# JaehaKim97/EDTR

Measured on AMD Instinct MI355X. Metric: restored 512x512 images/sec @ 4 denoise steps, higher is better.
Workload: dtype bf16; 1 GPU; EDTR-det s4 (sd21): vae_encode + q_sample(t=200) + 4 x (ControlNet+UNet) + vae_decode, batch 8/GPU of 512x512; global_batch=8, image_size=512, denoise_steps=4, parallelism=batch-sharded x1, graphs=True, batches_in_flight=2, precision=fast

## Files before the change

edtr_amd/csrc/igemm.hip:

```cpp
#include <stdlib.h>
#include <type_traits>
#include "common.h"

#ifdef EDTR_STAMPS
#define STAMP_VALUE 0
#define EDTR_STAMP(i)                                                                                                  \
    do {                                                                                                               \
        if (threadIdx.x == 0 && p.workspace && p.splitk <= 1) {                                                        \
            uint64_t* sb__ = static_cast<uint64_t*>(p.workspace) +                                                     \
                             (size_t)(blockIdx.x + gridDim.x * (blockIdx.y + gridDim.y * blockIdx.z)) * 16;             \
            if ((i) == 5) sb__[5] = (uint64_t)__builtin_amdgcn_s_getreg(63492) | ((uint64_t)__builtin_amdgcn_s_getreg(63508) << 32); \
            else if ((i) == 6 || (i) == 7) sb__[i] = __builtin_amdgcn_s_memrealtime();                             \
            else if ((i) >= 8) sb__[i] = (uint64_t)(STAMP_VALUE);                                             \
            else sb__[i] = __builtin_amdgcn_s_memtime();                                                               \
        }                                                                                                              \
    } while (0)
#define EDTR_STAMP_T(i)                                                                                                \
    do {                                                                                                               \
        if (threadIdx.x == 0 && p.workspace && p.splitk <= 1) {                                                        \
            uint64_t* sb__ = static_cast<uint64_t*>(p.workspace) +                                                     \
                             (size_t)(blockIdx.x + gridDim.x * (blockIdx.y + gridDim.y * blockIdx.z)) * 16;             \
            sb__[i] = __builtin_amdgcn_s_memtime();                                                                    \
        }                                                                                                              \
    } while (0)
// ... 1148 lines not shown
#pragma unroll
            for (int ni = 0; ni < NI; ++ni)
                bf[ni] = *reinterpret_cast<const U4*>(sw + tile_off(wn * 64 + ni * 32 + l31, c));
#pragma unroll
            for (int mi = 0; mi < MI; ++mi)
#pragma unroll
                for (int ni = 0; ni < NI; ++ni) acc[mi][ni] = T::mfma(af[mi], bf[ni], acc[mi][ni]);
        }
        asm volatile("s_waitcnt lgkmcnt(0)" ::: "memory");
#ifdef EDTR_STAMPS
        stamp_acc[3] += __builtin_amdgcn_s_memtime() - ts2;
#endif
        __builtin_amdgcn_s_barrier();
        asm volatile("" ::: "memory");
    }
    if (nkt == 0) __syncthreads();
    EDTR_STAMP(3);
#ifdef EDTR_STAMPS
#undef STAMP_VALUE
#define STAMP_VALUE stamp_acc[0]
    EDTR_STAMP(8);
#undef STAMP_VALUE
#define STAMP_VALUE stamp_acc[1]
    EDTR_STAMP(9);
#undef STAMP_VALUE
#define STAMP_VALUE stamp_acc[2]
    EDTR_STAMP(10);
#undef STAMP_VALUE
#define STAMP_VALUE stamp_acc[3]
    EDTR_STAMP(11);
#undef STAMP_VALUE
#define STAMP_VALUE 0
#endif
    tile_epilogue<T, MI, NI>(p, acc, smem, m0, n0, o_zoff);
    EDTR_STAMP(4); EDTR_STAMP(7);
}

template <typename T, bool SPATIAL, bool FAST>
int launch_dma(const edtr_igemm_params& p, hipStream_t stream) {
    constexpr int lds = 2 * (128 + 128) * BK * 2;
    static EdtrLdsOnce attr_set;
    if (int rc_ = edtr_lds_attr(reinterpret_cast<const void*>(&igemm_dma_kernel<T, SPATIAL, FAST>), lds, attr_set)) return rc_;
    const int nbm = (p.M + 127) / 128, nbn = (p.N + 127) / 128;
    dim3 grid(nbm * nbn, p.splitk > 1 ? p.splitk : 1, p.Z);
    hipLaunchKernelGGL((igemm_dma_kernel<T, SPATIAL, FAST>), grid, dim3(kThreads), lds, stream, p);
    EDTR_LAUNCH_CHECK();
    if (p.splitk > 1) return launch_splitk_reducer<T>(p, stream);
    return EDTR_OK;
}


struct KState { int t, tap, c0; };

template <typename T, bool SPATIAL>
__global__ void __launch_bounds__(512, 1) igemm_256_kernel(const edtr_igemm_params p) {
    constexpr int HALF = 128 * BK * 2;
    constexpr int BUF = 4 * HALF;
    extern __shared__ __attribute__((aligned(16))) char smem[];

    const int tid = threadIdx.x, lane = tid & 63, wave = __builtin_amdgcn_readfirstlane(tid >> 6);
    const int wr = wave >> 2, wc = wave & 3;
    const int l15 = lane & 15, lq = lane >> 4;

    const int nbm = (p.M + 255) / 256, nbn = (p.N + 255) / 256;
    int bid = blockIdx.x;
    {
        const int nblk = nbm * nbn, q = nblk >> 3, r = nblk & 7, x = bid & 7, j = bid >> 3;
        bid = (x < r ? x * (q + 1) : r * (q + 1) + (x - r) * q) + j;
    }
    int tm, tn;
    tile_coords(p, bid, nbm, nbn, tm, tn);
    const int m0 = tm * 256, n0 = tn * 256;

    const int z = blockIdx.z, zo = z / p.zdiv, zi = z - zo * p.zdiv;
    const int64_t a_zoff = zo * p.a_zs_outer + zi * p.a_zs_inner;
    const int64_t w_zoff = zo * p.w_zs_outer + zi * p.w_zs_inner;
    const int64_t o_zoff = zo * p.o_zs_outer + zi * p.o_zs_inner;
    const uint16_t* a1 = static_cast<const uint16_t*>(p.a1) + a_zoff;
    const uint16_t* wp = static_cast<const uint16_t*>(p.w) + w_zoff;
    const uint32_t smem_base = __builtin_amdgcn_readfirstlane(lds_addr_of(smem));

    const int rsub = lane >> 3, slot = lane & 7;
    const int Cin = p.C1;
    const int LH = p.upsample2x ? p.IH * 2 : p.IH, LW = p.upsample2x ? p.IW * 2 : p.IW;
    const int nvalid = p.n_valid > 0 ? p.n_valid : p.N;
    uint32_t voff_a[4], voff_w[4], a_mask[4], a_par[4];
    int b0 = 0, oy0 = 0, ox0 = 0;
    float rcp_ow = 0.0f, rcp_oh = 0.0f;
    if (SPATIAL) {
        const int hw = p.OH * p.OW;
        b0 = m0 / hw;
        const int rem0 = m0 - b0 * hw;
        oy0 = rem0 / p.OW;
        ox0 = rem0 - oy0 * p.OW;
        rcp_ow = 1.0f / (float)p.OW;
        rcp_oh = 1.0f / (float)p.OH;
    }
    const int64_t a_bias = SPATIAL ? ((int64_t)p.pad_t * p.IW + p.pad_l) * p.ld1 * 2 : 0;
    const u32x4 srd_a = make_srd(reinterpret_cast<const char*>(a1) - a_bias);
    const u32x4 srd_w = make_srd(wp);
#pragma unroll
    for (int q = 0; q < 4; ++q) {
        const int rih = wave * 16 + 8 * (q & 1) + rsub;
        const int row = (q >> 1) * 128 + rih;
        const int coff = (slot ^ ((rih >> 1) & 7)) * 8;
        const int m = m0 + row;
        const bool ok = m < p.M;
        uint32_t mask = 0;
        a_par[q] = 0;
        if (SPATIAL) {
            const int x = ox0 + row;
            int qx = (int)((float)x * rcp_ow), ox = x - qx * p.OW;
            if (ox >= p.OW) { ++qx; ox -= p.OW; }
            if (ox < 0) { --qx; ox += p.OW; }
            const int y = oy0 + qx;
            int qy = (int)((float)y * rcp_oh), oy = y - qy * p.OH;
            if (oy >= p.OH) { ++qy; oy -= p.OH; }
            if (oy < 0) { --qy; oy += p.OH; }
            const int iy0 = oy * p.stride - p.pad_t, ix0 = ox * p.stride - p.pad_l;
            const int ly = iy0 + p.pad_t, lx = ix0 + p.pad_l;
            const int sy = p.upsample2x ? ly >> 1 : ly, sx = p.upsample2x ? lx >> 1 : lx;
            a_par[q] = p.upsample2x ? (uint32_t)((ly & 1) | ((lx & 1) << 1)) : 0u;
            const int64_t pc = (int64_t)(b0 + qy) * p.IH * p.IW + (int64_t)sy * p.IW + sx;
            voff_a[q] = (uint32_t)((pc * p.ld1 + coff) * 2);
            if (p.taps == 9) {
                uint32_t rb = 0, cbits = 0;
#pragma unroll
                for (int k = 0; k < 3; ++k) {
                    const int iy = iy0 + k, ix = ix0 + k;
                    rb |= (iy >= 0 && iy < LH) ? (1u << (3 * k)) : 0u;
                    cbits |= (ix >= 0 && ix < LW) ? (1u << k) : 0u;
                }
                mask = ok ? rb * cbits : 0u;
            } else {
                mask = (ok && ly >= 0 && ly < LH && lx >= 0 && lx < LW) ? 1u : 0u;
            }
        } else {
            voff_a[q] = ok ? (uint32_t)(((int64_t)m * p.ld1 + coff) * 2) : kOobOffset;
            mask = 1u;
        }
        a_mask[q] = mask;
        const int n = n0 + row;
        voff_w[q] = n < nvalid ? (uint32_t)(((int64_t)n * p.ldw + coff) * 2) : kOobOffset;
    }

    const int nkt = p.K / BK;
    auto advance2 = [&](KState& s) {
        s.t += 2;
        if (SPATIAL) {
            s.tap += 2;
            while (s.tap >= p.taps) { s.tap -= p.taps; s.c0 += BK; }
        }
    };
    auto stage_half = [&](const KState& s, int buf, auto Hc) {
        constexpr int H = decltype(Hc)::value;
        const bool live = s.t < nkt;
        const uint32_t dst = smem_base + buf * BUF + H * HALF + wave * 2048;
        if constexpr (H < 2) {
            uint32_t soff = (uint32_t)s.t * (BK * 2), tapbit = 1u;
            uint32_t dy0 = 0, dy1 = 0, dx0 = 0, dx1 = 0;
            if (SPATIAL) {
                int ky = p.pad_t, kx = p.pad_l;
                if (p.taps == 9) { ky = (s.tap * 11) >> 5; kx = s.tap - 3 * ky; tapbit = 1u << s.tap; }
                if (p.upsample2x) {
                    const int rowb = p.IW * p.ld1 * 2, colb = p.ld1 * 2;
                    dy0 = (uint32_t)((((0 + ky - p.pad_t) >> 1) + p.pad_t) * rowb);
                    dy1 = (uint32_t)((((1 + ky - p.pad_t) >> 1) + p.pad_t) * rowb);
                    dx0 = (uint32_t)((((0 + kx - p.pad_l) >> 1) + p.pad_l) * colb);
                    dx1 = (uint32_t)((((1 + kx - p.pad_l) >> 1) + p.pad_l) * colb);
                    soff = (uint32_t)(s.c0 * 2);
                } else {
                    soff = (uint32_t)(((ky * p.IW + kx) * p.ld1 + s.c0) * 2);
                }
            }
            if (!live) tapbit = 0u;
#pragma unroll
            for (int j = 0; j < 2; ++j) {
                constexpr int q0 = H * 2;
                uint32_t vo = voff_a[q0 + j];
                if (SPATIAL && p.upsample2x) vo += ((a_par[q0 + j] & 1u) ? dy1 : dy0) + ((a_par[q0 + j] & 2u) ? dx1 : dx0);
                vo = (a_mask[q0 + j] & tapbit) ? vo : kOobOffset;
                dma16_buf(vo, srd_a, soff, dst + j * 1024);
            }
        } else {
            const uint32_t soff = SPATIAL ? (uint32_t)((s.tap * Cin + s.c0) * 2) : (uint32_t)s.t * (BK * 2);
#pragma unroll
            for (int j = 0; j < 2; ++j) {
                constexpr int q0 = (H - 2) * 2;
                const uint32_t vo = live ? voff_w[q0 + j] : kOobOffset;
                dma16_buf(vo, srd_w, soff, dst + j * 1024);
            }
        }
    };
    using H0 = std::integral_constant<int, 0>;
    using H1 = std::integral_constant<int, 1>;
    using H2 = std::integral_constant<int, 2>;
    using H3 = std::integral_constant<int, 3>;

    const int a_rd = tile_off(wr * 64 + l15, lq);
    const int b_rd = tile_off(wc * 32 + l15, lq);

    f32x4 acc[2][2][4][2];
#pragma unroll
    for (int i = 0; i < 2; ++i)
#pragma unroll
        for (int j = 0; j < 2; ++j)
#pragma unroll
            for (int a = 0; a < 4; ++a)
#pragma unroll
                for (int b = 0; b < 2; ++b) acc[i][j][a][b] = f32x4{0.0f, 0.0f, 0.0f, 0.0f};
    U4 afr[4][2], bfr[2][2][2];

    auto read_a = [&](int buf, int ah) {
        const char* base = smem + buf * BUF + ah * HALF;
#pragma unroll
        for (int mb = 0; mb < 4; ++mb) {
            afr[mb][0] = *reinterpret_cast<const U4*>(base + a_rd + mb * 2048);
            afr[mb][1] = *reinterpret_cast<const U4*>(base + (a_rd ^ 64) + mb * 2048);
        }
    };
    auto read_b = [&](int buf, auto BHc) {
        constexpr int BH = decltype(BHc)::value;
        const char* base = smem + buf * BUF + (2 + BH) * HALF;
#pragma unroll
        for (int nb = 0; nb < 2; ++nb) {
            bfr[BH][nb][0] = *reinterpret_cast<const U4*>(base + b_rd + nb * 2048);
            bfr[BH][nb][1] = *reinterpret_cast<const U4*>(base + (b_rd ^ 64) + nb * 2048);
        }
    };
    auto mma = [&](auto AHc, auto BHc) {
        constexpr int AH = decltype(AHc)::value, BH = decltype(BHc)::value;
#pragma unroll
        for (int ks = 0; ks < 2; ++ks)
#pragma unroll
            for (int mb = 0; mb < 4; ++mb)
#pragma unroll
                for (int nb = 0; nb < 2; ++nb) acc[AH][BH][mb][nb] = T::mfma16(afr[mb][ks], bfr[BH][nb][ks], acc[AH][BH][mb][nb]);
    };
    auto compute = [&](auto AHc, auto BHc) {
        asm volatile("s_waitcnt vmcnt(6)" ::: "memory");
        __builtin_amdgcn_s_barrier();
        asm volatile("s_waitcnt lgkmcnt(0)" ::: "memory");
        __builtin_amdgcn_sched_barrier(0);
        __builtin_amdgcn_s_setprio(1);
        mma(AHc, BHc);
        __builtin_amdgcn_s_setprio(0);
        __builtin_amdgcn_sched_barrier(0);
        __builtin_amdgcn_s_barrier();
        asm volatile("" ::: "memory");
    };

    KState sE{0, 0, 0}, sO{1, 1, 0};
    if (!SPATIAL || p.taps == 1) { sO.tap = 0; sO.c0 = BK; }
    stage_half(sE, 0, H0{}); stage_half(sE, 0, H1{}); stage_half(sE, 0, H2{}); stage_half(sE, 0, H3{});
    stage_half(sO, 1, H2{}); stage_half(sO, 1, H0{});
    advance2(sE);
    asm volatile("s_waitcnt vmcnt(4)" ::: "memory");
    __builtin_amdgcn_s_barrier();
    if (wr == 1) __builtin_amdgcn_s_barrier();
    asm volatile("" ::: "memory");

    const int niter = (nkt + 1) >> 1;
    for (int it = 0; it < niter; ++it) {
        read_b(0, H0{}); read_a(0, 0); stage_half(sO, 1, H3{}); compute(H0{}, H0{});
        read_b(0, H1{});               stage_half(sO, 1, H1{}); compute(H0{}, H1{}); advance2(sO);
        read_a(0, 1);                  stage_half(sE, 0, H2{}); compute(H1{}, H1{});
                                       stage_half(sE, 0, H0{}); compute(H1{}, H0{});
        read_b(1, H0{}); read_a(1, 0); stage_half(sE, 0, H3{}); compute(H0{}, H0{});
        read_b(1, H1{});               stage_half(sE, 0, H1{}); compute(H0{}, H1{}); advance2(sE);
        read_a(1, 1);                  stage_half(sO, 1, H2{}); compute(H1{}, H1{});
                                       stage_half(sO, 1, H0{}); compute(H1{}, H0{});
    }
    asm volatile("s_waitcnt vmcnt(0)" ::: "memory");
    if (wr == 0) __builtin_amdgcn_s_barrier();
    __syncthreads();

    float* stage = reinterpret_cast<float*>(smem);
    const bool gn_acc = p.gn_partial != nullptr && p.splitk <= 1;
    auto epilogue_pass = [&](auto HPc) {
        constexpr int h = decltype(HPc)::value;
#pragma unroll
        for (int bh = 0; bh < 2; ++bh)
#pragma unroll
            for (int mb = 0; mb < 4; ++mb)
#pragma unroll
                for (int nb = 0; nb < 2; ++nb)
#pragma unroll
                    for (int r = 0; r < 4; ++r)
                        stage[(wr * 64 + mb * 16 + 4 * lq + r) * 256 + bh * 128 + wc * 32 + nb * 16 + l15] = acc[h][bh][mb][nb][r];
        float gs[8], gq[8];
#pragma unroll
        for (int j = 0; j < 8; ++j) { gs[j] = 0.0f; gq[j] = 0.0f; }
        rows_phase<T, 128, 256, false, 512, 0, 256, false>(p, stage, m0 + h * 128, n0, p.N, o_zoff, gn_acc, gs, gq);
        __syncthreads();
        if (gn_acc) {
#pragma unroll
            for (int j = 0; j < 8; ++j) { gs[j] += __shfl_xor(gs[j], 32, 64); gq[j] += __shfl_xor(gq[j], 32, 64); }
            if (lane < 32) {
                float* dst = stage + (wave * 256 + lane * 8) * 2;
#pragma unroll
                for (int j = 0; j < 8; ++j) { dst[2 * j] = gs[j]; dst[2 * j + 1] = gq[j]; }
            }
            __syncthreads();
            if (tid < 256 && n0 + tid < p.N && m0 + h * 128 < p.M) {
                float a = 0.0f, q = 0.0f;
#pragma unroll
                for (int w = 0; w < 8; ++w) { a += stage[(w * 256 + tid) * 2]; q += stage[(w * 256 + tid) * 2 + 1]; }
                float* dst = p.gn_partial + ((int64_t)((m0 >> 7) + h) * gn_ld_of(p) + n0 + tid) * 2;
                dst[0] = a;
                dst[1] = q;
            }
            __syncthreads();
        }
    };
    epilogue_pass(H0{});
    epilogue_pass(H1{});
}

template <typename T, bool SPATIAL>
int launch_256(const edtr_igemm_params& p, hipStream_t stream) {
    constexpr int lds = 2 * 4 * 128 * BK * 2;
    static EdtrLdsOnce attr_set;
    if (int rc_ = edtr_lds_attr(reinterpret_cast<const void*>(&igemm_256_kernel<T, SPATIAL>), lds, attr_set)) return rc_;
    const int nbm = (p.M + 255) / 256, nbn = (p.N + 255) / 256;
    dim3 grid(nbm * nbn, 1, p.Z);
    hipLaunchKernelGGL((igemm_256_kernel<T, SPATIAL>), grid, dim3(512), lds, stream, p);
    EDTR_LAUNCH_CHECK();
    return EDTR_OK;
}

template <typename T, bool SPATIAL, int MB, int NB>
__global__ void __launch_bounds__(kThreads, 2) igemm_n160_kernel(const edtr_igemm_params p) {
    constexpr int BM = 32 * MB, BN = 32 * NB;
    constexpr int A_BYTES = BM * BK * 2, W_BYTES = BN * BK * 2, STAGE = A_BYTES + W_BYTES;
    extern __shared__ __attribute__((aligned(16))) char smem[];
    EDTR_STAMP(0); EDTR_STAMP(6); EDTR_STAMP(5);
    stagger_second_slot(p);

    const int tid = threadIdx.x, lane = tid & 63, wave = __builtin_amdgcn_readfirstlane(tid >> 6);
    const int wm = wave >> 1, wn = wave & 1;
    const int l15 = lane & 15, lq = lane >> 4;

    const int nbm = (p.M + BM - 1) / BM, nbn = (p.N + BN - 1) / BN;
    int bid = blockIdx.x;
    {
        const int nblk = nbm * nbn, q = nblk >> 3, r = nblk & 7, x = bid & 7, j = bid >> 3;
        bid = (x < r ? x * (q + 1) : r * (q + 1) + (x - r) * q) + j;
    }
    int tm, tn;
    tile_coords(p, bid, nbm, nbn, tm, tn);
    const int m0 = tm * BM, n0 = tn * BN;

    const int z = blockIdx.z, zo = z / p.zdiv, zi = z - zo * p.zdiv;
    const int64_t a_zoff = zo * p.a_zs_outer + zi * p.a_zs_inner;
    const int64_t w_zoff = zo * p.w_zs_outer + zi * p.w_zs_inner;
    const int64_t o_zoff = zo * p.o_zs_outer + zi * p.o_zs_inner;
    const uint16_t* a1 = static_cast<const uint16_t*>(p.a1) + a_zoff;
    const uint16_t* wp = static_cast<const uint16_t*>(p.w) + w_zoff;
    const uint32_t smem_base = __builtin_amdgcn_readfirstlane(lds_addr_of(smem));

    const int rsub = lane >> 3, slot = lane & 7;
    const int Cin = p.C1;
    const int LH = p.upsample2x ? p.IH * 2 : p.IH, LW = p.upsample2x ? p.IW * 2 : p.IW;
    const int nvalid = p.n_valid > 0 ? p.n_valid : p.N;
    uint32_t voff_a[MB], voff_w[NB], a_mask[MB], a_par[MB];
    int b0 = 0, oy0 = 0, ox0 = 0;
    float rcp_ow = 0.0f, rcp_oh = 0.0f;
    if (SPATIAL) {
        const int hw = p.OH * p.OW;
        b0 = m0 / hw;
        const int rem0 = m0 - b0 * hw;
        oy0 = rem0 / p.OW;
        ox0 = rem0 - oy0 * p.OW;
        rcp_ow = 1.0f / (float)p.OW;
        rcp_oh = 1.0f / (float)p.OH;
    }
    const int64_t a_bias = SPATIAL ? ((int64_t)p.pad_t * p.IW + p.pad_l) * p.ld1 * 2 : 0;
    const u32x4 srd_a = make_srd(reinterpret_cast<const char*>(a1) - a_bias);
    const u32x4 srd_w = make_srd(wp);
#pragma unroll
    for (int j = 0; j < MB; ++j) {
// ... 515 lines not shown
        __syncthreads();
        if (tid < 128 && n0 + tid < p.N) {
            float a = 0.0f, q = 0.0f;
#pragma unroll
            for (int w = 0; w < 8; ++w) { a += stage[(w * 128 + tid) * 2]; q += stage[(w * 128 + tid) * 2 + 1]; }
            float* dst = p.gn_partial + ((int64_t)(2 * tm) * gn_ld_of(p) + n0 + tid) * 2;
            dst[0] = a;
            dst[1] = q;
            dst[2 * gn_ld_of(p)] = 0.0f;
            dst[2 * gn_ld_of(p) + 1] = 0.0f;
        }
    }
    EDTR_STAMP(4); EDTR_STAMP(7);
}

template <typename T, int GEO>
int launch_halo(const edtr_igemm_params& p, hipStream_t stream) {
    constexpr bool UP2 = GEO == 1;
    constexpr int lds = UP2 ? 256 * 132 * 4 : (GEO == 2 ? 2 * 50 * 1024 + 3 * 128 * BK * 2 + 1024 : 2 * 48 * 1024 + 3 * 128 * BK * 2 + (GEO == 0 ? 2048 : 0));
    static EdtrLdsOnce attr_set;
    if (int rc_ = edtr_lds_attr(reinterpret_cast<const void*>(&igemm_halo_kernel<T, GEO>), lds, attr_set)) return rc_;
    const int nbm = GEO == 2 ? p.M >> 8 : (p.M / (p.OH * p.OW)) * (p.OH >> 4) * (p.OW >> 4), nbn = (p.N + 127) / 128;
    hipLaunchKernelGGL((igemm_halo_kernel<T, GEO>), dim3(nbm * nbn, p.splitk > 1 ? p.splitk : 1, 1), dim3(512), lds, stream, p);
    EDTR_LAUNCH_CHECK();
    if (p.splitk > 1) return launch_splitk_reducer<T>(p, stream);
    return EDTR_OK;
}

static bool igemm_halo_img8(const edtr_igemm_params& p) {
    return !p.upsample2x && p.OH == 8 && p.OW == 8 && p.IH == 8 && p.IW == 8 && (p.M & 255) == 0;
}

static bool igemm_halo_ok(const edtr_igemm_params& p, bool spatial) {
    const int up = p.upsample2x ? 2 : 1;
    if (p.upsample2x == 2 && ((p.IH & 15) || (p.IW & 15) || p.w_phase_stride < (int64_t)p.N * p.ldw || p.ldw < 4 * p.C1)) return false;
    return spatial && p.taps == 9 && p.stride == 1 && p.pad_t == 1 && p.pad_l == 1 && p.C2 == 0 && (p.C1 & 63) == 0 &&
           p.OH == p.IH * up && p.OW == p.IW * up && (((p.OH & 15) == 0 && (p.OW & 15) == 0) || igemm_halo_img8(p)) && p.Z == 1 &&
           p.splitk <= p.C1 / 64 && p.act != EDTR_ACT_GEGLU && p.M == (p.M / (p.OH * p.OW)) * p.OH * p.OW;
}

static bool igemm_fast_addressable(const edtr_igemm_params& p, bool spatial) {
    const int64_t a_rows = spatial ? (int64_t)(p.M / (p.OH * p.OW)) * p.IH * p.IW : p.M;
    const int64_t a_bytes = (a_rows + (spatial ? 3 * (int64_t)p.IW + 3 : 0)) * p.ld1 * 2 + (int64_t)p.K * 2;
    const int64_t w_bytes = (int64_t)p.N * p.ldw * 2 + (int64_t)p.K * 2;
    return a_bytes < 0xF0000000LL && w_bytes < 0xF0000000LL;
}

static int dbg_flags() {
    static int dbg = -1;
    if (dbg < 0) {
        const char* e8 = getenv("EDTR_IGEMM_GENERAL_EPILOGUE");
        const char* e10 = getenv("EDTR_IGEMM_N160_TWO_PASS");
        const char* e12 = getenv("EDTR_IGEMM_GEGLU_SERIAL");
        dbg = ((e8 && e8[0] == '1') ? 1 : 0) | ((e10 && e10[0] == '1') ? 2 : 0) | ((e12 && e12[0] == '1') ? 4 : 0);
    }
    return dbg;
}

template <typename T>
int dispatch(const edtr_igemm_params& p, int tile, bool spatial, hipStream_t s, bool dry) {
    if (tile == 20) {
        if (!spatial || !edtr_halo160_ok(p) || !igemm_fast_addressable(p, spatial)) return EDTR_E_UNSUPPORTED;
        if (dry) return tile;
        return edtr_launch_halo160(p, s);
    }
    if (tile == 21) {
        if (!spatial || !edtr_halo512p_ok(p) || !igemm_fast_addressable(p, spatial)) return EDTR_E_UNSUPPORTED;
        if (dry) return tile;
        return edtr_launch_halo512p(p, s);
    }
    if (tile == 17) {
        if (!spatial || !edtr_halo512_ok(p) || !igemm_fast_addressable(p, spatial)) return EDTR_E_UNSUPPORTED;
        if (dry) return tile;
        return edtr_launch_halo512(p, s);
    }
    if (tile == 16) {
        if (!igemm_halo_ok(p, spatial) || !igemm_fast_addressable(p, spatial)) return EDTR_E_UNSUPPORTED;
        if (dry) return tile;
        if (igemm_halo_img8(p)) return launch_halo<T, 2>(p, s);
        if (p.upsample2x == 2) return launch_halo<T, 3>(p, s);
        return p.upsample2x ? launch_halo<T, 1>(p, s) : launch_halo<T, 0>(p, s);
    }
    if (tile >= 3 && tile <= 14) {
        const bool fast = (!p.upsample2x || (p.stride == 1 && (tile == 3 || tile >= 6))) && igemm_fast_addressable(p, spatial);
        if (tile == 14) {
            if (!fast || p.act == EDTR_ACT_GEGLU || p.gn_partial) return EDTR_E_UNSUPPORTED;
            if (dry) return tile;
            return spatial ? launch_n160<T, true, 8, 1>(p, s) : launch_n160<T, false, 8, 1>(p, s);
        }
        if (tile == 8) {
            if (!fast || p.act == EDTR_ACT_GEGLU) return EDTR_E_UNSUPPORTED;
            if (dry) return tile;
            return spatial ? launch_n160<T, true, 4, 5>(p, s) : launch_n160<T, false, 4, 5>(p, s);
        }
        if (tile == 6) {
            if (!fast || p.splitk > 1 || p.act == EDTR_ACT_GEGLU) return EDTR_E_UNSUPPORTED;
            if (dry) return tile;
            return spatial ? launch_256<T, true>(p, s) : launch_256<T, false>(p, s);
        }
        if (dry) return tile;
        if (!spatial) return fast ? launch_dma<T, false, true>(p, s) : launch_dma<T, false, false>(p, s);
        return fast ? launch_dma<T, true, true>(p, s) : launch_dma<T, true, false>(p, s);
    }
    if (dry) return tile;
    if (tile == 1) return spatial ? launch<T, 2, 2, true>(p, s) : launch<T, 2, 2, false>(p, s);
    return spatial ? launch<T, 1, 1, true>(p, s) : launch<T, 1, 1, false>(p, s);
}

}

namespace {
__global__ void __launch_bounds__(256) gn_finalize_kernel(const float* partial, int tiles_per_image, int C, int groups,
                                                         double* sums) {
    __shared__ double red_s[256], red_q[256];
    const int g = blockIdx.x, b = blockIdx.y, cpg = C / groups;
    const int total = tiles_per_image * cpg;
    double s = 0.0, q = 0.0;
    for (int i = threadIdx.x; i < total; i += 256) {
        const int t = i / cpg, c = g * cpg + (i - t * cpg);
        const float* src = partial + (((int64_t)b * tiles_per_image + t) * C + c) * 2;
        s += (double)src[0];
        q += (double)src[1];
    }
    red_s[threadIdx.x] = s;
    red_q[threadIdx.x] = q;
    __syncthreads();
    for (int o = 128; o > 0; o >>= 1) {
        if (threadIdx.x < o) { red_s[threadIdx.x] += red_s[threadIdx.x + o]; red_q[threadIdx.x] += red_q[threadIdx.x + o]; }
        __syncthreads();
    }
    if (threadIdx.x == 0) {
        sums[((int64_t)b * groups + g) * 2] = red_s[0];
        sums[((int64_t)b * groups + g) * 2 + 1] = red_q[0];
    }
}
}

extern "C" int edtr_gn_finalize(const float* partial, int tiles_per_image, int B, int C, int groups, double* sums,
                                edtr_stream_t stream) {
    if (!partial || !sums) return EDTR_E_NULL;
    if (tiles_per_image <= 0 || B <= 0 || C <= 0 || groups <= 0 || C % groups) return EDTR_E_SHAPE;
    hipLaunchKernelGGL(gn_finalize_kernel, dim3(groups, B), dim3(256), 0, static_cast<hipStream_t>(stream), partial,
                       tiles_per_image, C, groups, sums);
    EDTR_LAUNCH_CHECK();
    return EDTR_OK;
}

namespace {
__global__ void __launch_bounds__(256) gn_table_kernel(const float* partial, int tiles_per_image, const double* sums, int C, int groups,
                                                      int HW, const float* gamma, const float* beta, float eps, float* table) {
    __shared__ double red_s[256], red_q[256];
    const int g = blockIdx.x, b = blockIdx.y, cpg = C / groups;
    double s = 0.0, q = 0.0;
    if (partial) {
        const int total = tiles_per_image * cpg;
// ... 72 lines not shown
        return EDTR_E_ALIGN;
    if ((p.a_zs_outer & 7) || (p.a_zs_inner & 7) || (p.w_zs_outer & 7) || (p.w_zs_inner & 7) ||
        (p.o_zs_outer & 3) || (p.o_zs_inner & 3))
        return EDTR_E_ALIGN;
    if ((p.bias_n && !aligned16(p.bias_n)) || (p.rowvec && (!aligned16(p.rowvec) || (p.rowvec_ld & 3)))) return EDTR_E_ALIGN;
    if (p.n_valid < 0 || p.n_valid > p.N) return EDTR_E_SHAPE;
    if (p.residual && p.Z != 1) return EDTR_E_UNSUPPORTED;
    if (p.rowvec && p.Z != 1) return EDTR_E_UNSUPPORTED;
    if (p.splitk < 0) return EDTR_E_SHAPE;
    if (p.splitk <= 1) p.splitk = 1;
    if (p.splitk > 1) {
        if (p.Z != 1 || p.act == EDTR_ACT_GEGLU) return EDTR_E_UNSUPPORTED;
        if (!p.workspace) return EDTR_E_NULL;
        if (p.workspace_bytes < (int64_t)p.splitk * p.M * p.N * 4 || !aligned16(p.workspace)) return EDTR_E_SHAPE;
        if (p.splitk > (p.K + 63) / 64) return EDTR_E_SHAPE;
    }

    if (p.vt_out) {
        if (p.Z != 1 || p.splitk > 1 || p.act == EDTR_ACT_GEGLU || p.residual || p.rowvec || p.gn_partial || p.out_f32 || spatial)
            return EDTR_E_UNSUPPORTED;
        if (p.rows_per_image <= 0 || (p.rows_per_image & 7) || (p.M & 7) || p.vt_col0 <= 0 || p.vt_col0 >= p.N) return EDTR_E_SHAPE;
        if ((p.vt_ld & 7) || p.vt_ld < p.rows_per_image || !aligned16(p.vt_out)) return EDTR_E_ALIGN;
    }

    if (p.row_stats) {
        if (p.Z != 1 || p.splitk > 1 || p.act == EDTR_ACT_GEGLU || p.vt_out) return EDTR_E_UNSUPPORTED;
        if (p.N & 31) return EDTR_E_SHAPE;
        if (!aligned16(p.row_stats)) return EDTR_E_ALIGN;
    }
    if (p.ln_stats) {
        if (p.Z != 1 || p.splitk > 1 || p.taps != 1 || spatial || p.C2) return EDTR_E_UNSUPPORTED;
        if (!p.ln_c1 || !p.ln_c2) return EDTR_E_NULL;
        if (p.ln_slots <= 0 || p.ln_slots * 32 != p.K || p.ln_C <= 0 || p.ln_C > p.K) return EDTR_E_SHAPE;
        if (!aligned16(p.ln_stats) || !aligned16(p.ln_c1) || !aligned16(p.ln_c2)) return EDTR_E_ALIGN;
    }

    const bool dma_ok = p.C2 == 0 && (p.C1 & 63) == 0;
    int tile = p.tile;
    if (tile == 0) {
        const int64_t big = (int64_t)((p.M + 127) / 128) * ((p.N + 127) / 128) * p.Z;
        tile = dma_ok ? 3 : (big >= 200 ? 1 : 2);
        const int nbn256 = (p.N + 255) / 256;
        const int64_t nb256 = (int64_t)((p.M + 255) / 256) * nbn256 * p.Z;
        static int no_auto = -1;
        if (no_auto < 0) {
            const char* e = getenv("EDTR_IGEMM_NO_AUTO");
            no_auto = e ? atoi(e) : 0;
        }
        const bool pp_ok = dma_ok && p.splitk <= 1 && p.act != EDTR_ACT_GEGLU && (!p.upsample2x || p.stride == 1) &&
                           igemm_fast_addressable(p, spatial);
        const int64_t nb160 = (int64_t)((p.M + 127) / 128) * (p.N / 160) * p.Z;
        if (pp_ok && !(no_auto & (1 << 8)) && p.N % 160 == 0 && nb160 >= 200 && (p.N % 128 != 0 || p.K >= 640))
            tile = 8;
        else if (pp_ok && !(no_auto & (1 << 6)) && p.K >= 1024 && nb256 >= 120 && p.N * 5 >= nbn256 * 256 * 4)
            tile = 6;
        static int halo = -1;
        if (halo < 0) {
            const char* e4 = getenv("EDTR_IGEMM_HALO");
            halo = (e4 && e4[0] == '0') ? 0 : 1;
        }
        if (halo && dma_ok && (p.N & 127) == 0 && igemm_halo_ok(p, spatial) && igemm_fast_addressable(p, spatial) &&
            (int64_t)(p.M >> 8) * (p.N >> 7) * p.splitk >= 48)
            tile = 16;
        static int ragged = -1;
        if (ragged < 0) {
            const char* e6 = getenv("EDTR_IGEMM_HALO_RAGGED");
            ragged = (e6 && e6[0] == '0') ? 0 : 1;
        }
        if (halo && ragged && dma_ok && (p.N & 127) != 0 && p.N > 128 && p.splitk <= 1 && igemm_halo_ok(p, spatial) &&
            igemm_fast_addressable(p, spatial)) {
            const int64_t units = (int64_t)(p.M >> 8) * ((p.N + 127) >> 7);
            if (units >= 48 && units <= 256) tile = 16;
        }
        static int skinny = -1;
        if (skinny < 0) {
            const char* e3 = getenv("EDTR_IGEMM_SKINNY");
            skinny = (e3 && e3[0] == '0') ? 0 : 1;
        }
        if (skinny && tile == 3 && p.N <= 32 && p.M >= 65536 && p.splitk <= 1 && !p.gn_partial && p.act != EDTR_ACT_GEGLU &&
            (!p.upsample2x || p.stride == 1) && igemm_fast_addressable(p, spatial))
            tile = 14;
    }
    static int halo512 = -1;
    if (halo512 < 0) {
        const char* e5 = getenv("EDTR_IGEMM_HALO512");
        halo512 = e5 ? atoi(e5) : 1;
    }
    const bool h512_ok = spatial && (p.C1 & 31) == 0 && edtr_halo512_ok(p) && igemm_fast_addressable(p, spatial);
    const int cus = dry ? 256 : edtr_cu_count();
    if (p.tile == 0 && tile == 16 && halo512 > 0 && h512_ok && (int64_t)(p.M >> 9) * (p.N >> 7) >= (int64_t)cus * halo512) tile = 17;
    static int halo512p = -1;
    if (halo512p < 0) {
        const char* e13 = getenv("EDTR_IGEMM_HALO512P");
        halo512p = e13 ? atoi(e13) : 0;
    }
    if (p.tile == 0 && tile == 17 && halo512p > 0 && edtr_halo512p_ok(p) && (int64_t)(p.M >> 9) * (p.N >> 7) >= (int64_t)cus * halo512p) tile = 21;
    static int halo160 = -1;
    if (halo160 < 0) {
        const char* e10 = getenv("EDTR_IGEMM_HALO160");
        halo160 = (e10 && e10[0] == '0') ? 0 : 1;
    }
    if (p.tile == 0 && tile == 8 && halo160 && spatial && edtr_halo160_ok(p) && igemm_fast_addressable(p, spatial)) {
        const int64_t units = (int64_t)(p.M >> 8) * (p.N / 160), tail = units % cus, most = (int64_t)cus * 3 / 4;
        if (units >= most && (tail == 0 || tail >= most)) tile = 20;
    }
    if (p.a_gn) {
        if (p.tile == 21 || (p.tile == 0 && tile == 21)) {
            if (!h512_ok || !edtr_halo512p_ok(p)) return EDTR_E_UNSUPPORTED;
            tile = 21;
        } else if (p.tile == 17 || (p.tile == 0 && tile == 17)) {
            if (!h512_ok) return EDTR_E_UNSUPPORTED;
            tile = 17;
        } else {
            if ((p.dtype != EDTR_BF16 && p.dtype != EDTR_F16) || !spatial || p.upsample2x || !dma_ok || !igemm_halo_ok(p, spatial) ||
                igemm_halo_img8(p) || !igemm_fast_addressable(p, spatial) || (p.tile != 0 && p.tile != 16))
                return EDTR_E_UNSUPPORTED;
            tile = 16;
        }
        if (!aligned16(p.a_gn)) return EDTR_E_ALIGN;
    }
    if (p.out16) {
        if (!p.out_f32 || p.Z != 1 || p.act == EDTR_ACT_GEGLU || p.vt_out) return EDTR_E_UNSUPPORTED;
        if ((p.ld16 & 7) || !aligned16(p.out16)) return EDTR_E_ALIGN;
    }
    if (p.a_wrap != 0) {
        if (p.a_wrap < 0 || p.K != 2 * p.a_wrap || (p.a_wrap & 63) || spatial || p.taps != 1 || p.C2 || p.Z != 1 || p.ln_stats) return EDTR_E_UNSUPPORTED;
        if (p.tile != 0 && !(p.tile == 1 || p.tile == 2 || p.tile == 3 || p.tile == 8)) return EDTR_E_UNSUPPORTED;
        if (!(tile == 1 || tile == 2 || tile == 3 || tile == 8)) tile = 3;
    }
    if (p.upsample2x == 2) {
        if (p.tile != 0 && p.tile != 16) return EDTR_E_UNSUPPORTED;
        if (!dma_ok || !igemm_halo_ok(p, spatial) || !igemm_fast_addressable(p, spatial)) return EDTR_E_UNSUPPORTED;
        tile = 16;
    }
    if (p.vt_out) {
        if (p.tile == 0 && !((tile == 8 && p.vt_col0 % 160 == 0) || ((tile == 1 || tile == 3) && p.vt_col0 % 128 == 0)))
            tile = (dma_ok && p.N % 160 == 0 && p.vt_col0 % 160 == 0 && igemm_fast_addressable(p, spatial)) ? 8
                   : (p.vt_col0 % 128 == 0 ? (dma_ok ? 3 : 1) : -1);
        const int bn = tile == 8 ? 160 : 128;
        if (!(tile == 1 || tile == 3 || tile == 8) || p.vt_col0 % bn != 0) return EDTR_E_UNSUPPORTED;
    }
    if (p.ln_stats && !(tile == 1 || tile == 3)) {
        if (p.tile != 0) return EDTR_E_UNSUPPORTED;
        tile = dma_ok ? 3 : 1;
        if (p.vt_out && p.vt_col0 % 128 != 0) return EDTR_E_UNSUPPORTED;
    }
    if (p.row_stats && !(tile == 1 || tile == 2 || tile == 3 || (tile == 8 && !(dbg_flags() & 2)))) {
        if (p.tile != 0) return EDTR_E_UNSUPPORTED;
        tile = dma_ok ? 3 : 1;
    }
    if ((p.row_stats || p.vt_out) && (tile == 16 || tile == 17 || tile == 20 || tile == 21)) return EDTR_E_UNSUPPORTED;
    if (p.act == EDTR_ACT_GEGLU && tile == 2) tile = 1;
    if (tile >= 3 && !dma_ok && !((tile == 17 || tile == 20 || tile == 21) && p.C2 == 0 && (p.C1 & 31) == 0)) return EDTR_E_UNSUPPORTED;
    if (p.gn_partial) {
        const int sr = p.gn_slot_rows > 0 ? p.gn_slot_rows : 128;
        if (p.gn_ld < 0 || (p.gn_ld > 0 && p.gn_ld < p.N)) return EDTR_E_SHAPE;
        if (p.Z != 1 || p.act == EDTR_ACT_GEGLU) return EDTR_E_UNSUPPORTED;
        if (p.splitk > 1) {
            if ((sr != 64 && sr != 128) || p.M % sr || (p.N & 31)) return EDTR_E_UNSUPPORTED;
        } else if (tile == 2 || sr != 128 || (p.M & 127)) {
            return EDTR_E_UNSUPPORTED;
        }
    }
    if (!(tile == 1 || tile == 2 || tile == 3 || tile == 6 || tile == 8 || tile == 14 || tile == 16 || tile == 17 || tile == 20 || tile == 21)) return EDTR_E_DTYPE;
    p.debug_flags = dbg_flags();
    p.stagger = 0;
    if ((tile == 3 || tile == 8) && p.splitk <= 1) {
        static int pct = -1;
        if (pct < 0) {
            const char* e7 = getenv("EDTR_IGEMM_STAGGER");
            pct = e7 ? atoi(e7) : 0;
        }
        const int bm = 128, bn = tile == 8 ? 160 : 128;
        const int64_t wgs = (int64_t)((p.M + bm - 1) / bm) * ((p.N + bn - 1) / bn) * p.Z;
        const int nkt = (p.K + 63) / 64;
        if (pct > 0 && wgs >= 768 && nkt <= 48) {
            const int life = 4000 + nkt * 1350 + (p.act == EDTR_ACT_GEGLU ? 11000 : 9000);
            p.stagger = (int)((int64_t)life * pct / 200);
        }
    }
    hipStream_t s = static_cast<hipStream_t>(stream);
    return p.dtype == EDTR_BF16 ? dispatch<BF16>(p, tile, spatial, s, dry) : dispatch<F16>(p, tile, spatial, s, dry);
}

extern "C" int edtr_igemm(const edtr_igemm_params* pp, edtr_stream_t stream) { return igemm_run(pp, stream, false); }

extern "C" int edtr_igemm_plan(const edtr_igemm_params* pp) { return igemm_run(pp, nullptr, true); }
```

Measured before the change: 122.2 images/s.

## Add 256x128 ping-pong igemm tile, GEGLU epilogue, and tuned vmcnt waits

Generalizes the 256x256 ping-pong GEMM kernel to a BN template, adding a 256x128 variant (tile 22). The auto-selector picks it for dense 1x1 GEMMs whose 256x128 block count fills between half and one full wave of CUs. It also lets tile 6 handle GEGLU with a fused gate epilogue and vt_out outputs. Per-stage vmcnt waits are now derived from the tile shape rather than fixed, with an env drain fallback. The aim is better CU occupancy and fewer tail waves for mid-sized GEMMs, at the cost of more kernel variants and more complex selection heuristics.

```diff
diff --git a/edtr_amd/csrc/igemm.hip b/edtr_amd/csrc/igemm.hip
--- a/edtr_amd/csrc/igemm.hip
+++ b/edtr_amd/csrc/igemm.hip
@@ -1224,17 +1224,33 @@
 
 struct KState { int t, tap, c0; };
 
-template <typename T, bool SPATIAL>
+template <int N>
+__device__ __forceinline__ void wait_vm() {
+    static_assert(N == 0 || N == 3 || N == 4 || N == 5 || N == 6, "wait_vm: add the count");
+    if constexpr (N == 0) asm volatile("s_waitcnt vmcnt(0)" ::: "memory");
+    else if constexpr (N == 3) asm volatile("s_waitcnt vmcnt(3)" ::: "memory");
+    else if constexpr (N == 4) asm volatile("s_waitcnt vmcnt(4)" ::: "memory");
+    else if constexpr (N == 5) asm volatile("s_waitcnt vmcnt(5)" ::: "memory");
+    else asm volatile("s_waitcnt vmcnt(6)" ::: "memory");
+}
+
+template <typename T, bool SPATIAL, int BN, bool DRAIN>
 __global__ void __launch_bounds__(512, 1) igemm_256_kernel(const edtr_igemm_params p) {
+    static_assert(BN == 256 || BN == 128, "igemm_256_kernel: 256 x 256 or 256 x 128");
     constexpr int HALF = 128 * BK * 2;
-    constexpr int BUF = 4 * HALF;
+    constexpr int HALF_B = BN / 2 * BK * 2;
+    constexpr int BUF = 2 * HALF + 2 * HALF_B;
+    constexpr int WR = BN == 256 ? 2 : 4, MB = 128 / (16 * WR);
+    constexpr int DB = BN / 128;
+    constexpr int VM_B = DRAIN ? 0 : 2 * DB + 2, VM_A = DRAIN ? 0 : 4 + DB, VM_PRO = DRAIN ? 0 : DB + 2;
     extern __shared__ __attribute__((aligned(16))) char smem[];
 
     const int tid = threadIdx.x, lane = tid & 63, wave = __builtin_amdgcn_readfirstlane(tid >> 6);
-    const int wr = wave >> 2, wc = wave & 3;
+    const int wr = wave / (8 / WR), wc = wave % (8 / WR);
     const int l15 = lane & 15, lq = lane >> 4;
-
-    const int nbm = (p.M + 255) / 256, nbn = (p.N + 255) / 256;
+    const int bcol = (wc >> 1) * 64 + (wc & 1) * 16;
+
+    const int nbm = (p.M + 255) / 256, nbn = (p.N + BN - 1) / BN;
     int bid = blockIdx.x;
     {
         const int nblk = nbm * nbn, q = nblk >> 3, r = nblk & 7, x = bid & 7, j = bid >> 3;
@@ -1242,7 +1258,7 @@
     }
     int tm, tn;
     tile_coords(p, bid, nbm, nbn, tm, tn);
-    const int m0 = tm * 256, n0 = tn * 256;
+    const int m0 = tm * 256, n0 = tn * BN;
 
     const int z = blockIdx.z, zo = z / p.zdiv, zi = z - zo * p.zdiv;
     const int64_t a_zoff = zo * p.a_zs_outer + zi * p.a_zs_inner;
@@ -1256,7 +1272,7 @@
     const int Cin = p.C1;
     const int LH = p.upsample2x ? p.IH * 2 : p.IH, LW = p.upsample2x ? p.IW * 2 : p.IW;
     const int nvalid = p.n_valid > 0 ? p.n_valid : p.N;
-    uint32_t voff_a[4], voff_w[4], a_mask[4], a_par[4];
+    uint32_t voff_a[4], voff_w[2 * DB], a_mask[4], a_par[4];
     int b0 = 0, oy0 = 0, ox0 = 0;
     float rcp_ow = 0.0f, rcp_oh = 0.0f;
     if (SPATIAL) {
@@ -1312,7 +1328,12 @@
             mask = 1u;
         }
         a_mask[q] = mask;
-        const int n = n0 + row;
+    }
+#pragma unroll
+    for (int q = 0; q < 2 * DB; ++q) {
+        const int rih = wave * 8 * DB + 8 * (q % DB) + rsub;
+        const int coff = (slot ^ ((rih >> 1) & 7)) * 8;
+        const int n = n0 + (q / DB) * (BN / 2) + rih;
         voff_w[q] = n < nvalid ? (uint32_t)(((int64_t)n * p.ldw + coff) * 2) : kOobOffset;
     }
 
@@ -1327,8 +1348,8 @@
     auto stage_half = [&](const KState& s, int buf, auto Hc) {
         constexpr int H = decltype(Hc)::value;
         const bool live = s.t < nkt;
-        const uint32_t dst = smem_base + buf * BUF + H * HALF + wave * 2048;
         if constexpr (H < 2) {
+            const uint32_t dst = smem_base + buf * BUF + H * HALF + wave * 2048;
             uint32_t soff = (uint32_t)s.t * (BK * 2), tapbit = 1u;
             uint32_t dy0 = 0, dy1 = 0, dx0 = 0, dx1 = 0;
             if (SPATIAL) {
@@ -1355,10 +1376,11 @@
                 dma16_buf(vo, srd_a, soff, dst + j * 1024);
             }
         } else {
+            const uint32_t dst = smem_base + buf * BUF + 2 * HALF + (H - 2) * HALF_B + wave * (1024 * DB);
             const uint32_t soff = SPATIAL ? (uint32_t)((s.tap * Cin + s.c0) * 2) : (uint32_t)s.t * (BK * 2);
 #pragma unroll
-            for (int j = 0; j < 2; ++j) {
-                constexpr int q0 = (H - 2) * 2;
+            for (int j = 0; j < DB; ++j) {
+                constexpr int q0 = (H - 2) * DB;
                 const uint32_t vo = live ? voff_w[q0 + j] : kOobOffset;
                 dma16_buf(vo, srd_w, soff, dst + j * 1024);
             }
@@ -1369,35 +1391,35 @@
     using H2 = std::integral_constant<int, 2>;
     using H3 = std::integral_constant<int, 3>;
 
-    const int a_rd = tile_off(wr * 64 + l15, lq);
-    const int b_rd = tile_off(wc * 32 + l15, lq);
-
-    f32x4 acc[2][2][4][2];
+    const int a_rd = tile_off(wr * 16 * MB + l15, lq);
+    const int b_rd = tile_off(bcol + l15, lq);
+
+    f32x4 acc[2][2][MB][2];
 #pragma unroll
     for (int i = 0; i < 2; ++i)
 #pragma unroll
         for (int j = 0; j < 2; ++j)
 #pragma unroll
-            for (int a = 0; a < 4; ++a)
+            for (int a = 0; a < MB; ++a)
 #pragma unroll
                 for (int b = 0; b < 2; ++b) acc[i][j][a][b] = f32x4{0.0f, 0.0f, 0.0f, 0.0f};
-    U4 afr[4][2], bfr[2][2][2];
+    U4 afr[MB][2], bfr[2][2][2];
 
     auto read_a = [&](int buf, int ah) {
         const char* base = smem + buf * BUF + ah * HALF;
 #pragma unroll
-        for (int mb = 0; mb < 4; ++mb) {
+        for (int mb = 0; mb < MB; ++mb) {
             afr[mb][0] = *reinterpret_cast<const U4*>(base + a_rd + mb * 2048);
             afr[mb][1] = *reinterpret_cast<const U4*>(base + (a_rd ^ 64) + mb * 2048);
         }
     };
     auto read_b = [&](int buf, auto BHc) {
         constexpr int BH = decltype(BHc)::value;
-        const char* base = smem + buf * BUF + (2 + BH) * HALF;
+        const char* base = smem + buf * BUF + 2 * HALF + BH * HALF_B;
 #pragma unroll
         for (int nb = 0; nb < 2; ++nb) {
-            bfr[BH][nb][0] = *reinterpret_cast<const U4*>(base + b_rd + nb * 2048);
-            bfr[BH][nb][1] = *reinterpret_cast<const U4*>(base + (b_rd ^ 64) + nb * 2048);
+            bfr[BH][nb][0] = *reinterpret_cast<const U4*>(base + b_rd + nb * 4096);
+            bfr[BH][nb][1] = *reinterpret_cast<const U4*>(base + (b_rd ^ 64) + nb * 4096);
         }
     };
     auto mma = [&](auto AHc, auto BHc) {
@@ -1405,12 +1427,12 @@
 #pragma unroll
         for (int ks = 0; ks < 2; ++ks)
 #pragma unroll
-            for (int mb = 0; mb < 4; ++mb)
+            for (int mb = 0; mb < MB; ++mb)
 #pragma unroll
                 for (int nb = 0; nb < 2; ++nb) acc[AH][BH][mb][nb] = T::mfma16(afr[mb][ks], bfr[BH][nb][ks], acc[AH][BH][mb][nb]);
     };
-    auto compute = [&](auto AHc, auto BHc) {
-        asm volatile("s_waitcnt vmcnt(6)" ::: "memory");
+    auto compute = [&](auto AHc, auto BHc, auto VMc) {
+        wait_vm<decltype(VMc)::value>();
         __builtin_amdgcn_s_barrier();
         asm volatile("s_waitcnt lgkmcnt(0)" ::: "memory");
         __builtin_amdgcn_sched_barrier(0);
@@ -1421,51 +1443,83 @@
         __builtin_amdgcn_s_barrier();
         asm volatile("" ::: "memory");
     };
-
+    using VB = std::integral_constant<int, VM_B>;
+    using VA = std::integral_constant<int, VM_A>;
+
+    const bool late = wave >= 4;
     KState sE{0, 0, 0}, sO{1, 1, 0};
     if (!SPATIAL || p.taps == 1) { sO.tap = 0; sO.c0 = BK; }
     stage_half(sE, 0, H0{}); stage_half(sE, 0, H1{}); stage_half(sE, 0, H2{}); stage_half(sE, 0, H3{});
     stage_half(sO, 1, H2{}); stage_half(sO, 1, H0{});
     advance2(sE);
-    asm volatile("s_waitcnt vmcnt(4)" ::: "memory");
+    wait_vm<VM_PRO>();
     __builtin_amdgcn_s_barrier();
-    if (wr == 1) __builtin_amdgcn_s_barrier();
+    if (late) __builtin_amdgcn_s_barrier();
     asm volatile("" ::: "memory");
 
     const int niter = (nkt + 1) >> 1;
     for (int it = 0; it < niter; ++it) {
-        read_b(0, H0{}); read_a(0, 0); stage_half(sO, 1, H3{}); compute(H0{}, H0{});
-        read_b(0, H1{});               stage_half(sO, 1, H1{}); compute(H0{}, H1{}); advance2(sO);
-        read_a(0, 1);                  stage_half(sE, 0, H2{}); compute(H1{}, H1{});
-                                       stage_half(sE, 0, H0{}); compute(H1{}, H0{});
-        read_b(1, H0{}); read_a(1, 0); stage_half(sE, 0, H3{}); compute(H0{}, H0{});
-        read_b(1, H1{});               stage_half(sE, 0, H1{}); compute(H0{}, H1{}); advance2(sE);
-        read_a(1, 1);                  stage_half(sO, 1, H2{}); compute(H1{}, H1{});
-                                       stage_half(sO, 1, H0{}); compute(H1{}, H0{});
+        read_b(0, H0{}); read_a(0, 0); stage_half(sO, 1, H3{}); compute(H0{}, H0{}, VB{});
+        read_b(0, H1{});               stage_half(sO, 1, H1{}); compute(H0{}, H1{}, VA{}); advance2(sO);
+        read_a(0, 1);                  stage_half(sE, 0, H2{}); compute(H1{}, H1{}, VB{});
+                                       stage_half(sE, 0, H0{}); compute(H1{}, H0{}, VA{});
+        read_b(1, H0{}); read_a(1, 0); stage_half(sE, 0, H3{}); compute(H0{}, H0{}, VB{});
+        read_b(1, H1{});               stage_half(sE, 0, H1{}); compute(H0{}, H1{}, VA{}); advance2(sE);
+        read_a(1, 1);                  stage_half(sO, 1, H2{}); compute(H1{}, H1{}, VB{});
+                                       stage_half(sO, 1, H0{}); compute(H1{}, H0{}, VA{});
     }
     asm volatile("s_waitcnt vmcnt(0)" ::: "memory");
-    if (wr == 0) __builtin_amdgcn_s_barrier();
+    if (!late) __builtin_amdgcn_s_barrier();
     __syncthreads();
 
     float* stage = reinterpret_cast<float*>(smem);
-    const bool gn_acc = p.gn_partial != nullptr && p.splitk <= 1;
+    const bool geglu = p.act == EDTR_ACT_GEGLU;
+    const bool gn_acc = BN == 256 && p.gn_partial != nullptr && p.splitk <= 1;
     auto epilogue_pass = [&](auto HPc) {
         constexpr int h = decltype(HPc)::value;
-#pragma unroll
-        for (int bh = 0; bh < 2; ++bh)
-#pragma unroll
-            for (int mb = 0; mb < 4; ++mb)
-#pragma unroll
-                for (int nb = 0; nb < 2; ++nb)
-#pragma unroll
-                    for (int r = 0; r < 4; ++r)
-                        stage[(wr * 64 + mb * 16 + 4 * lq + r) * 256 + bh * 128 + wc * 32 + nb * 16 + l15] = acc[h][bh][mb][nb][r];
         float gs[8], gq[8];
 #pragma unroll
         for (int j = 0; j < 8; ++j) { gs[j] = 0.0f; gq[j] = 0.0f; }
-        rows_phase<T, 128, 256, false, 512, 0, 256, false>(p, stage, m0 + h * 128, n0, p.N, o_zoff, gn_acc, gs, gq);
+        if (geglu) {
+            constexpr int BNO = BN / 2;
+#pragma unroll
+            for (int bh = 0; bh < 2; ++bh) {
+                const int nv = n0 + bh * (BN / 2) + bcol + l15;
+                const bool nok = p.bias_n && nv < p.N;
+                const float bv = nok ? p.bias_n[nv] : 0.0f, bg = nok ? p.bias_n[nv + 32] : 0.0f;
+                const int oc = bh * (BN / 4) + (wc >> 1) * 32 + (wc & 1) * 16 + l15;
+#pragma unroll
+                for (int g = 0; g < MB / 2; ++g) {
+                    float val[8], gate[8];
+#pragma unroll
+                    for (int e = 0; e < 8; ++e) {
+                        const int mb = 2 * g + (e >> 2), r = e & 3;
+                        val[e] = acc[h][bh][mb][0][r] * p.alpha + bv;
+                        gate[e] = acc[h][bh][mb][1][r] * p.alpha + bg;
+                    }
+                    gelu_erf_lockstep<false>(gate);
+#pragma unroll
+                    for (int e = 0; e < 8; ++e) {
+                        const int mb = 2 * g + (e >> 2), r = e & 3;
+                        stage[(wr * 16 * MB + mb * 16 + 4 * lq + r) * BNO + oc] = val[e] * gate[e];
+                    }
+                }
+            }
+            rows_phase<T, 128, BNO, true, 512, 0, BNO, false>(p, stage, m0 + h * 128, n0 / 2, p.N / 2, o_zoff, false, gs, gq);
+        } else {
+#pragma unroll
+            for (int bh = 0; bh < 2; ++bh)
+#pragma unroll
+                for (int mb = 0; mb < MB; ++mb)
+#pragma unroll
+                    for (int nb = 0; nb < 2; ++nb)
+#pragma unroll
+                        for (int r = 0; r < 4; ++r)
+                            stage[(wr * 16 * MB + mb * 16 + 4 * lq + r) * BN + bh * (BN / 2) + bcol + nb * 32 + l15] = acc[h][bh][mb][nb][r];
+            rows_phase<T, 128, BN, false, 512, 0, BN, false>(p, stage, m0 + h * 128, n0, p.N, o_zoff, gn_acc, gs, gq);
+        }
         __syncthreads();
-        if (gn_acc) {
+        if (BN == 256 && gn_acc) {
 #pragma unroll
             for (int j = 0; j < 8; ++j) { gs[j] += __shfl_xor(gs[j], 32, 64); gq[j] += __shfl_xor(gq[j], 32, 64); }
             if (lane < 32) {
@@ -1489,16 +1543,22 @@
     epilogue_pass(H1{});
 }
 
-template <typename T, bool SPATIAL>
-int launch_256(const edtr_igemm_params& p, hipStream_t stream) {
-    constexpr int lds = 2 * 4 * 128 * BK * 2;
+template <typename T, bool SPATIAL, int BN, bool DRAIN>
+static int launch_256_as(const edtr_igemm_params& p, hipStream_t stream) {
+    constexpr int lds = 2 * (2 * 128 + BN) * BK * 2;
     static EdtrLdsOnce attr_set;
-    if (int rc_ = edtr_lds_attr(reinterpret_cast<const void*>(&igemm_256_kernel<T, SPATIAL>), lds, attr_set)) return rc_;
-    const int nbm = (p.M + 255) / 256, nbn = (p.N + 255) / 256;
+    if (int rc_ = edtr_lds_attr(reinterpret_cast<const void*>(&igemm_256_kernel<T, SPATIAL, BN, DRAIN>), lds, attr_set)) return rc_;
+    const int nbm = (p.M + 255) / 256, nbn = (p.N + BN - 1) / BN;
     dim3 grid(nbm * nbn, 1, p.Z);
-    hipLaunchKernelGGL((igemm_256_kernel<T, SPATIAL>), grid, dim3(512), lds, stream, p);
+    hipLaunchKernelGGL((igemm_256_kernel<T, SPATIAL, BN, DRAIN>), grid, dim3(512), lds, stream, p);
     EDTR_LAUNCH_CHECK();
     return EDTR_OK;
+}
+
+template <typename T, int BN>
+int launch_256(const edtr_igemm_params& p, bool spatial, hipStream_t stream) {
+    if (p.debug_flags & 8) return spatial ? launch_256_as<T, true, BN, true>(p, stream) : launch_256_as<T, false, BN, true>(p, stream);
+    return spatial ? launch_256_as<T, true, BN, false>(p, stream) : launch_256_as<T, false, BN, false>(p, stream);
 }
 
 template <typename T, bool SPATIAL, int MB, int NB>
@@ -2120,7 +2180,9 @@
         const char* e8 = getenv("EDTR_IGEMM_GENERAL_EPILOGUE");
         const char* e10 = getenv("EDTR_IGEMM_N160_TWO_PASS");
         const char* e12 = getenv("EDTR_IGEMM_GEGLU_SERIAL");
-        dbg = ((e8 && e8[0] == '1') ? 1 : 0) | ((e10 && e10[0] == '1') ? 2 : 0) | ((e12 && e12[0] == '1') ? 4 : 0);
+        const char* e14 = getenv("EDTR_IGEMM_PP_DRAIN");
+        dbg = ((e8 && e8[0] == '1') ? 1 : 0) | ((e10 && e10[0] == '1') ? 2 : 0) | ((e12 && e12[0] == '1') ? 4 : 0) |
+              ((e14 && e14[0] == '1') ? 8 : 0);
     }
     return dbg;
 }
@@ -2162,13 +2224,19 @@
             return spatial ? launch_n160<T, true, 4, 5>(p, s) : launch_n160<T, false, 4, 5>(p, s);
         }
         if (tile == 6) {
-            if (!fast || p.splitk > 1 || p.act == EDTR_ACT_GEGLU) return EDTR_E_UNSUPPORTED;
+            if (!fast || p.splitk > 1) return EDTR_E_UNSUPPORTED;
             if (dry) return tile;
-            return spatial ? launch_256<T, true>(p, s) : launch_256<T, false>(p, s);
+            return launch_256<T, 256>(p, spatial, s);
         }
         if (dry) return tile;
         if (!spatial) return fast ? launch_dma<T, false, true>(p, s) : launch_dma<T, false, false>(p, s);
         return fast ? launch_dma<T, true, true>(p, s) : launch_dma<T, true, false>(p, s);
+    }
+    if (tile == 22) {
+        const bool fast = (!p.upsample2x || p.stride == 1) && igemm_fast_addressable(p, spatial);
+        if (!fast || p.splitk > 1 || p.gn_partial) return EDTR_E_UNSUPPORTED;
+        if (dry) return tile;
+        return launch_256<T, 128>(p, spatial, s);
     }
     if (dry) return tile;
     if (tile == 1) return spatial ? launch<T, 2, 2, true>(p, s) : launch<T, 2, 2, false>(p, s);
@@ -2347,8 +2415,17 @@
         const int64_t nb160 = (int64_t)((p.M + 127) / 128) * (p.N / 160) * p.Z;
         if (pp_ok && !(no_auto & (1 << 8)) && p.N % 160 == 0 && nb160 >= 200 && (p.N % 128 != 0 || p.K >= 640))
             tile = 8;
-        else if (pp_ok && !(no_auto & (1 << 6)) && p.K >= 1024 && nb256 >= 120 && p.N * 5 >= nbn256 * 256 * 4)
+        else if (pp_ok && !(no_auto & (1 << 6)) && p.K >= 1024 && nb256 >= 120 && p.N * 5 >= nbn256 * 256 * 4 && !p.vt_out)
             tile = 6;
+        if (pp_ok && !(no_auto & (1 << 22)) && !spatial && p.taps == 1 && !p.gn_partial && !p.row_stats && !p.ln_stats && p.a_wrap == 0 && (tile == 3 || tile == 8)) {
+            const int cus_pp = dry ? 256 : edtr_cu_count();
+            const int64_t nb22 = (int64_t)((p.M + 255) / 256) * ((p.N + 127) / 128) * p.Z, tail6 = nb256 % cus_pp;
+            if (!(no_auto & (1 << 6)) && p.vt_out && p.vt_col0 % 256 == 0 && nb256 >= cus_pp &&
+                (tail6 == 0 || 4 * tail6 >= 3 * cus_pp))
+                tile = 6;
+            else if (p.N % 128 == 0 && (!p.vt_out || p.vt_col0 % 128 == 0) && 2 * nb22 >= cus_pp && nb22 <= cus_pp)
+                tile = 22;
+        }
         static int halo = -1;
         if (halo < 0) {
             const char* e4 = getenv("EDTR_IGEMM_HALO");
@@ -2429,11 +2506,12 @@
         tile = 16;
     }
     if (p.vt_out) {
-        if (p.tile == 0 && !((tile == 8 && p.vt_col0 % 160 == 0) || ((tile == 1 || tile == 3) && p.vt_col0 % 128 == 0)))
+        const int bn = tile == 8 ? 160 : tile == 6 ? 256 : 128;
+        if (p.tile == 0 && !((tile == 1 || tile == 3 || tile == 6 || tile == 8 || tile == 22) && p.vt_col0 % bn == 0))
             tile = (dma_ok && p.N % 160 == 0 && p.vt_col0 % 160 == 0 && igemm_fast_addressable(p, spatial)) ? 8
                    : (p.vt_col0 % 128 == 0 ? (dma_ok ? 3 : 1) : -1);
-        const int bn = tile == 8 ? 160 : 128;
-        if (!(tile == 1 || tile == 3 || tile == 8) || p.vt_col0 % bn != 0) return EDTR_E_UNSUPPORTED;
+        const int bn2 = tile == 8 ? 160 : tile == 6 ? 256 : 128;
+        if (!(tile == 1 || tile == 3 || tile == 6 || tile == 8 || tile == 22) || p.vt_col0 % bn2 != 0) return EDTR_E_UNSUPPORTED;
     }
     if (p.ln_stats && !(tile == 1 || tile == 3)) {
         if (p.tile != 0) return EDTR_E_UNSUPPORTED;
@@ -2457,8 +2535,9 @@
             return EDTR_E_UNSUPPORTED;
         }
     }
-    if (!(tile == 1 || tile == 2 || tile == 3 || tile == 6 || tile == 8 || tile == 14 || tile == 16 || tile == 17 || tile == 20 || tile == 21)) return EDTR_E_DTYPE;
-    p.debug_flags = dbg_flags();
+    if (!(tile == 1 || tile == 2 || tile == 3 || tile == 6 || tile == 8 || tile == 14 || tile == 16 || tile == 17 || tile == 20 || tile == 21 || tile == 22))
+        return EDTR_E_DTYPE;
+    p.debug_flags = dbg_flags() | (p.debug_flags & 8);
     p.stagger = 0;
     if ((tile == 3 || tile == 8) && p.splitk <= 1) {
         static int pct = -1;
```

Measured after the change: 122.2 images/s (median of 4 runs). No clear change (+0.0%).
